# CNR-STIIMA-IRAS/rosdyn

Hardware: AMD Instinct MI355X
Metric: RNEA+regressor evals/s (6-DOF, batch 1e6) (higher is better)
Workload: dtype f64; 1 GPU; configs[1]: 6-DOF chain (ur10_like base_link->wrist_3_link, n=6, P=60), batch 1000000 samples per GPU, fp64 getJointTorque + dense getRegressor, inputs sample-major, Y layout stacked; samples_per_gpu=1000000, n_active=6, n_params=60, parallelism=sample-sharded x1

## Files before the change

### rosdyn_amd/csrc/rdyn_kernels.hip

```cpp
#include <hip/hip_runtime.h>
#include <type_traits>
#include "rdyn_device.h"
#include "rdyn_devmath.h"
#include "rdyn_kernels.h"
#include "rdyn_record_stage.h"

namespace
{

enum
{
  MODE_REGRESSOR = 0,
  MODE_TORQUE = 1,
  MODE_INERTIA = 2,
  MODE_REGRESSOR_GRAM = 3,
  MODE_REGRESSOR_EXPAND = 4,
  MODE_REGRESSOR_EXPAND_STAGED = 5
};
#define RDYN_IS_EXPAND(MODE) ((MODE) == MODE_REGRESSOR_EXPAND || (MODE) == MODE_REGRESSOR_EXPAND_STAGED)
#define RDYN_IS_REGRESSOR(MODE) ((MODE) == MODE_REGRESSOR || (MODE) == MODE_REGRESSOR_GRAM || RDYN_IS_EXPAND(MODE))
#define RDYN_BODY_EXIT return

#ifdef RDYN_LOCAL_WAVES
#define RDYN_LOCAL_ATTR __attribute__((amdgpu_waves_per_eu(RDYN_LOCAL_WAVES, RDYN_LOCAL_WAVES)))
#else
#define RDYN_LOCAL_ATTR
#endif
template <int NJ, int MODE>
__global__ __launch_bounds__(256) RDYN_LOCAL_ATTR void k_local_sweep(const RdynSweepArgs a)
{
  const unsigned blk = blockIdx.x;
  constexpr double* expand_tile = nullptr;
#include "rdyn_local_sweep_body.inc"
}
template <int NJ, int MODE>
__global__ __launch_bounds__(64) RDYN_LOCAL_ATTR void k_local_sweep_rec(const RdynSweepArgs a)
{
  const unsigned blk = blockIdx.x;
  constexpr double* expand_tile = nullptr;
#define RDYN_LOCAL_WGS 64
#include "rdyn_local_sweep_body.inc"
}
#ifndef RDYN_EXPAND_WAVES
#define RDYN_EXPAND_WAVES 2
#endif
template <int NJ>
__global__ __launch_bounds__(64) __attribute__((amdgpu_waves_per_eu(RDYN_EXPAND_WAVES, RDYN_EXPAND_WAVES))) void k_expand_staged(const RdynSweepArgs a)
{
  constexpr int MODE = MODE_REGRESSOR_EXPAND_STAGED;
  extern __shared__ __attribute__((aligned(16))) double expand_tile[];
  const unsigned blk = blockIdx.x;
#include "rdyn_local_sweep_body.inc"
}

template <int NJ, int MODE>
__global__ __launch_bounds__(256) void k_local_sweep_multi(const RdynSweepArgs* __restrict__ table)
{
#pragma clang diagnostic push
#pragma clang diagnostic ignored "-Wold-style-cast"
  const RDYN_CONST_AS RdynSweepArgs& a = *((const RDYN_CONST_AS RdynSweepArgs*)table + blockIdx.y);
#pragma clang diagnostic pop
  const unsigned blk = blockIdx.x;
  constexpr double* expand_tile = nullptr;
#include "rdyn_local_sweep_body.inc"
}

template <int NJ, int LEVEL, bool STAGED, class Args>
__device__ __forceinline__ void base_sweep_body(const Args& a, const int64_t s, char* lds = nullptr)
{
  ChainPtr c = as_const(a.chain);
  const int lane = threadIdx.x & 63;
  bool stg = false;
  RecordRing<96> ringT;
  RecordRing<48> ringV, ringA;
  char* small_area = nullptr;
  if constexpr (STAGED)
  {
    const int64_t s_wave = s - lane;
    stg = a.n_samples - s_wave >= 64;
    if (stg)
    {
      char* p = lds;
      if (a.T_links)
      {
        ringT.init(p, a.T_links + s_wave * a.tl_ss, 96u * (NJ + 1), lane);
        p += RecordRing<96>::BYTES;
      }
      if (LEVEL >= 2 && a.twists)
      {
        ringV.init(p, a.twists + s_wave * a.tw_ss, 48u * (NJ + 1), lane);
        p += RecordRing<48>::BYTES;
      }
      if (LEVEL >= 3 && a.dtwists)
      {
        ringA.init(p, a.dtwists + s_wave * a.tw_ss, 48u * (NJ + 1), lane);
        p += RecordRing<48>::BYTES;
      }
      small_area = p;
    }
  }
  if (s >= a.n_samples) return;
  const double* __restrict__ qp = a.q + s * a.in_ss;
  const double* __restrict__ dqp = (LEVEL >= 2 && a.dq) ? a.dq + s * a.in_ss : nullptr;
  const double* __restrict__ ddqp = (LEVEL >= 3 && a.ddq) ? a.ddq + s * a.in_ss : nullptr;
  const int64_t es = a.out_se;

  double R[9] = {1, 0, 0, 0, 1, 0, 0, 0, 1};
  V3 p = mk(0, 0, 0);
  V3 vlin = mk(0, 0, 0), vang = mk(0, 0, 0), alin = mk(0, 0, 0), aang = mk(0, 0, 0);

  auto put3x4 = [&](double* __restrict__ o) {
#pragma unroll
    for (int cc = 0; cc < 3; ++cc)
#pragma unroll
      for (int r = 0; r < 3; ++r) o[(int64_t)(cc * 3 + r) * es] = R[r * 3 + cc];
    o[9 * es] = p.x;
    o[10 * es] = p.y;
    o[11 * es] = p.z;
  };
  auto put6 = [&](double* __restrict__ o, V3 l, V3 g) {
    o[0] = l.x; o[es] = l.y; o[2 * es] = l.z; o[3 * es] = g.x; o[4 * es] = g.y; o[5 * es] = g.z;
  };

  auto frame_out = [&](const int link) {
    if (!a.T_links) return;
    if (STAGED && stg)
    {
#pragma unroll
      for (int cc = 0; cc < 3; ++cc)
#pragma unroll
        for (int r = 0; r < 3; ++r) ringT.put((uint32_t)(96 * link + 8 * (cc * 3 + r)), R[r * 3 + cc]);
      ringT.put((uint32_t)(96 * link + 72), p.x);
      ringT.put((uint32_t)(96 * link + 80), p.y);
      ringT.put((uint32_t)(96 * link + 88), p.z);
      ringT.flush(96 * link, 96 * (link + 1));
    }
    else
      put3x4(a.T_links + s * a.tl_ss + (int64_t)(12 * link) * es);
  };
  auto six_out = [&](const RecordRing<48>& ring, double* base, const int link, V3 l, V3 g) {
    if (STAGED && stg)
    {
      ring.put((uint32_t)(48 * link), l.x);
      ring.put((uint32_t)(48 * link + 8), l.y);
      ring.put((uint32_t)(48 * link + 16), l.z);
      ring.put((uint32_t)(48 * link + 24), g.x);
      ring.put((uint32_t)(48 * link + 32), g.y);
      ring.put((uint32_t)(48 * link + 40), g.z);
      ring.flush(48 * link, 48 * (link + 1));
    }
    else
      put6(base + s * a.tw_ss + (int64_t)(6 * link) * es, l, g);
  };
  V3 pref = mk(0, 0, 0);
  int j_up = 0;
  const bool jst = LEVEL == 1 && STAGED && stg && a.J;
  SmallRecords smJ;
  V3 zs[(LEVEL == 1 && STAGED) ? NJ : 1], pos[(LEVEL == 1 && STAGED) ? NJ : 1];
  if (LEVEL == 1 && !STAGED && a.J)
  {
    double R1[9] = {1, 0, 0, 0, 1, 0, 0, 0, 1};
    V3 p1 = mk(0, 0, 0);
#pragma unroll
    for (int l = 0; l < NJ; ++l)
    {
      JointRef J = c->j[l];
      if (l < a.j_link)
      {
        if (J.in_idx >= 0) ++j_up;
        const double ql = J.in_idx >= 0 ? qp[J.in_idx * a.in_sj] : 0.0;
        double Rpc[9];
        V3 t = ld3(J.t);
        if (J.type == RDYN_REVOLUTE)
        {
          double sn, cs;
          rdyn_sincos(ql, &sn, &cs);
          const double oc = 1.0 - cs;
#pragma unroll
          for (int i = 0; i < 9; ++i) Rpc[i] = fma(sn, J.B[i], fma(oc, J.C[i], J.A[i]));
        }
        else
        {
#pragma unroll
          for (int i = 0; i < 9; ++i) Rpc[i] = J.A[i];
          if (J.type == RDYN_PRISMATIC) t = axpy(t, ld3(J.up), ql);
        }
        p1 = p1 + rot(R1, t);
        double Rn[9];
#pragma unroll
        for (int r = 0; r < 3; ++r)
#pragma unroll
          for (int cc = 0; cc < 3; ++cc)
            Rn[r * 3 + cc] = fma(R1[r * 3 + 0], Rpc[cc], fma(R1[r * 3 + 1], Rpc[3 + cc], R1[r * 3 + 2] * Rpc[6 + cc]));
#pragma unroll
        for (int i = 0; i < 9; ++i) R1[i] = Rn[i];
      }
    }
    pref = p1;
  }
  frame_out(0);
  if (LEVEL >= 2 && a.twists) six_out(ringV, a.twists, 0, vlin, vang);
  if (LEVEL >= 3 && a.dtwists) six_out(ringA, a.dtwists, 0, alin, aang);

#pragma unroll
  for (int f = 0; f < NJ; ++f)
  {
    JointRef J = c->j[f];
    const int type = J.type;
    const int idx = J.in_idx;
    double qf = 0.0, dqf = 0.0, ddqf = 0.0;
    if (idx >= 0)
    {
      const int64_t o = idx * a.in_sj;
      qf = qp[o];
      if (LEVEL >= 2 && dqp) dqf = dqp[o];
      if (LEVEL >= 3 && ddqp) ddqf = ddqp[o];
    }
    double Rpc[9];
    V3 t = ld3(J.t);
    if (type == RDYN_REVOLUTE)
    {
      double sn, cs;
      rdyn_sincos(qf, &sn, &cs);
      const double oc = 1.0 - cs;
#pragma unroll
      for (int i = 0; i < 9; ++i) Rpc[i] = fma(sn, J.B[i], fma(oc, J.C[i], J.A[i]));
    }
    else
    {
#pragma unroll
      for (int i = 0; i < 9; ++i) Rpc[i] = J.A[i];
      if (type == RDYN_PRISMATIC) t = axpy(t, ld3(J.up), qf);
    }
    const V3 zl = LEVEL >= 1 ? rot(R, ld3(J.up)) : mk(0, 0, 0);
    const V3 d = rot(R, t);
    double Rn[9];
#pragma unroll
    for (int r = 0; r < 3; ++r)
#pragma unroll
      for (int cc = 0; cc < 3; ++cc)
        Rn[r * 3 + cc] = fma(R[r * 3 + 0], Rpc[cc], fma(R[r * 3 + 1], Rpc[3 + cc], R[r * 3 + 2] * Rpc[6 + cc]));
#pragma unroll
    for (int i = 0; i < 9; ++i) R[i] = Rn[i];
    p = p + d;
    if (LEVEL == 1 && STAGED)
    {
      zs[(LEVEL == 1 && STAGED) ? f : 0] = zl;
      pos[(LEVEL == 1 && STAGED) ? f : 0] = p;
    }
    if (LEVEL == 1 && !STAGED && a.J && idx >= 0)
    {
      V3 jlin = mk(0, 0, 0), jang = mk(0, 0, 0);
      if (idx < j_up)
      {
        if (type == RDYN_REVOLUTE)
        {
          jlin = cross(zl, pref - p);
          jang = zl;
        }
        else if (type == RDYN_PRISMATIC)
          jlin = zl;
      }
      put6(a.J + s * a.j_ss + (int64_t)(6 * idx) * es, jlin, jang);
    }
    if (LEVEL >= 2)
    {
      V3 Sl = mk(0, 0, 0), Sa = mk(0, 0, 0);
      if (type == RDYN_REVOLUTE) Sa = zl;
      else if (type == RDYN_PRISMATIC) Sl = zl;
      const V3 nvl = axpy(vlin + cross(vang, d), Sl, dqf);
      const V3 nva = axpy(vang, Sa, dqf);
      if (LEVEL >= 3)
      {
        const V3 cl = cross(nva, Sl) + cross(nvl, Sa);
        const V3 ca = cross(nva, Sa);
        alin = axpy(axpy(alin + cross(aang, d), cl, dqf), Sl, ddqf);
        aang = axpy(axpy(aang, ca, dqf), Sa, ddqf);
      }
      vlin = nvl;
      vang = nva;
    }
    frame_out(f + 1);
    if (LEVEL >= 2 && a.twists) six_out(ringV, a.twists, f + 1, vlin, vang);
    if (LEVEL >= 3 && a.dtwists) six_out(ringA, a.dtwists, f + 1, alin, aang);
  }
  if (STAGED && stg)
  {
    if (a.T_links) ringT.finish();
    if (LEVEL >= 2 && a.twists) ringV.finish();
    if (LEVEL >= 3 && a.dtwists) ringA.finish();
  }
  SmallRecords sm;
  if (a.T_bt)
  {
    if (STAGED && stg)
    {
      sm.init(small_area, 12, lane);
#pragma unroll
      for (int cc = 0; cc < 3; ++cc)
#pragma unroll
        for (int r = 0; r < 3; ++r) sm.put(cc * 3 + r, R[r * 3 + cc]);
      sm.put(9, p.x);
      sm.put(10, p.y);
      sm.put(11, p.z);
      sm.copy_out(a.T_bt + (s - lane) * a.tb_ss, lane);
    }
    else
      put3x4(a.T_bt + s * a.tb_ss);
  }
  if constexpr (LEVEL == 1 && STAGED)
  {
    if (a.J)
    {
      if (jst) smJ.init(small_area, 6 * c->n_active, lane);
      V3 pr = p;
      int up = 0;
#pragma unroll
      for (int l = 0; l < NJ; ++l)
      {
        if (a.j_link == l + 1) pr = pos[l];
        if (l < a.j_link && c->j[l].in_idx >= 0) ++up;
      }
      if (a.j_link == 0) pr = mk(0, 0, 0);
#pragma unroll
      for (int l = 0; l < NJ; ++l)
      {
        const int k = c->j[l].in_idx;
        if (k < 0) continue;
        const int ty = c->j[l].type;
        V3 jlin = mk(0, 0, 0), jang = mk(0, 0, 0);
        if (k < up)
        {
          if (ty == RDYN_REVOLUTE)
          {
            jlin = cross(zs[l], pr - pos[l]);
            jang = zs[l];
          }
          else if (ty == RDYN_PRISMATIC)
            jlin = zs[l];
        }
        if (jst)
        {
          smJ.put(6 * k, jlin.x); smJ.put(6 * k + 1, jlin.y); smJ.put(6 * k + 2, jlin.z);
          smJ.put(6 * k + 3, jang.x); smJ.put(6 * k + 4, jang.y); smJ.put(6 * k + 5, jang.z);
        }
        else
          put6(a.J + s * a.j_ss + (int64_t)(6 * k) * es, jlin, jang);
      }
      if (jst) smJ.copy_out(a.J + (s - lane) * a.j_ss, lane);
    }
  }
}

template <int NJ, int LEVEL>
__global__ __launch_bounds__(256) void k_base_sweep(const RdynKinArgs a)
{
  base_sweep_body<NJ, LEVEL, false>(a, (int64_t)blockIdx.x * 256 + threadIdx.x);
}
template <int NJ, int LEVEL>
__global__ __launch_bounds__(64) void k_base_sweep_staged(const RdynKinArgs a)
{
  extern __shared__ __attribute__((aligned(16))) char stage_lds[];
  base_sweep_body<NJ, LEVEL, true>(a, (int64_t)blockIdx.x * 64 + threadIdx.x, stage_lds);
}

template <int NJ>
__global__ __launch_bounds__(256) void k_sample_all(const RdynAllArgs all)
{
  const unsigned blk = blockIdx.x;
  constexpr double* expand_tile = nullptr;
  switch (blockIdx.y)
  {
  case 0:
    if (all.frames.T_bt || all.frames.T_links) base_sweep_body<NJ, 0, false>(all.frames, (int64_t)blk * 256 + threadIdx.x);
    return;
  case 1:
    if (all.jacobian.J) base_sweep_body<NJ, 1, false>(all.jacobian, (int64_t)blk * 256 + threadIdx.x);
    return;
  case 2:
    if (all.twists.dtwists) base_sweep_body<NJ, 3, false>(all.twists, (int64_t)blk * 256 + threadIdx.x);
    else if (all.twists.twists) base_sweep_body<NJ, 2, false>(all.twists, (int64_t)blk * 256 + threadIdx.x);
    return;
  case 3:
  {
    if (!all.torque.tau) return;
    constexpr int MODE = MODE_TORQUE;
    const RdynSweepArgs& a = all.torque;
#include "rdyn_local_sweep_body.inc"
    return;
  }
  case 4:
  {
    if (!all.torque_nl.tau) return;
    constexpr int MODE = MODE_TORQUE;
    const RdynSweepArgs& a = all.torque_nl;
#include "rdyn_local_sweep_body.inc"
    return;
  }
  case 5:
  {
    if (!all.inertia.M) return;
    constexpr int MODE = MODE_INERTIA;
    const RdynSweepArgs& a = all.inertia;
#include "rdyn_local_sweep_body.inc"
    return;
  }
  default:
  {
    if (!all.regressor.Y) return;
    constexpr int MODE = MODE_REGRESSOR;
    const RdynSweepArgs& a = all.regressor;
#include "rdyn_local_sweep_body.inc"
    return;
  }
  }
}

template <int NJ>
hipError_t launch_local_nj(int mode, const RdynSweepArgs& a, hipStream_t st)
{
  const unsigned grid = (unsigned)((a.n_samples + 255) / 256);
  switch (mode)
  {
  case MODE_REGRESSOR_EXPAND_STAGED:
    hipLaunchKernelGGL((k_expand_staged<NJ>), dim3((unsigned)((a.n_samples + 63) / 64)), dim3(64), (size_t)64 * (RDYN_EXPAND_TILE_COLS(NJ) * NJ + 2 + 3 * NJ + 1) * sizeof(double), st, a);
    break;
  case MODE_REGRESSOR: hipLaunchKernelGGL((k_local_sweep<NJ, MODE_REGRESSOR>), dim3(grid), dim3(256), 0, st, a); break;
  case MODE_REGRESSOR_GRAM: hipLaunchKernelGGL((k_local_sweep<NJ, MODE_REGRESSOR_GRAM>), dim3(grid), dim3(256), 0, st, a); break;
  case MODE_REGRESSOR_EXPAND: hipLaunchKernelGGL((k_local_sweep<NJ, MODE_REGRESSOR_EXPAND>), dim3(grid), dim3(256), 0, st, a); break;
  case MODE_TORQUE:
    if (a.staged) hipLaunchKernelGGL((k_local_sweep_rec<NJ, MODE_TORQUE>), dim3((unsigned)((a.n_samples + 63) / 64)), dim3(64), (size_t)64 * (a.staged | 1) * 8, st, a);
    else hipLaunchKernelGGL((k_local_sweep<NJ, MODE_TORQUE>), dim3(grid), dim3(256), 0, st, a);
    break;
  default:
    if (a.staged) hipLaunchKernelGGL((k_local_sweep_rec<NJ, MODE_INERTIA>), dim3((unsigned)((a.n_samples + 63) / 64)), dim3(64), (size_t)32 * (a.staged | 1) * 8, st, a);
    else hipLaunchKernelGGL((k_local_sweep<NJ, MODE_INERTIA>), dim3(grid), dim3(256), 0, st, a);
    break;
  }
  return hipGetLastError();
}
constexpr size_t kFramesStageLds = 33 * 1024;
template <int NJ>
hipError_t launch_base_nj(const RdynKinArgs& a, hipStream_t st)
{
  if (a.staged)
  {
    size_t lds = 0, small = 0;
    if (a.T_links) lds += RecordRing<96>::BYTES;
    if (a.twists) lds += RecordRing<48>::BYTES;
    if (a.dtwists) lds += RecordRing<48>::BYTES;
    if (a.T_bt) small = (size_t)64 * 13 * 8;
    if (a.J && (size_t)64 * (size_t)((6 * a.n_active) | 1) * 8 > small) small = (size_t)64 * (size_t)((6 * a.n_active) | 1) * 8;
    lds += small;
    if (a.T_links && lds < kFramesStageLds) lds = kFramesStageLds;
#ifdef RDYN_STAGE_LDS_PAD
    lds += RDYN_STAGE_LDS_PAD;
#endif
    const unsigned g64 = (unsigned)((a.n_samples + 63) / 64);
    if (a.dtwists) hipLaunchKernelGGL((k_base_sweep_staged<NJ, 3>), dim3(g64), dim3(64), lds, st, a);
    else if (a.twists) hipLaunchKernelGGL((k_base_sweep_staged<NJ, 2>), dim3(g64), dim3(64), lds, st, a);
    else if (a.J) hipLaunchKernelGGL((k_base_sweep_staged<NJ, 1>), dim3(g64), dim3(64), lds, st, a);
    else hipLaunchKernelGGL((k_base_sweep_staged<NJ, 0>), dim3(g64), dim3(64), lds, st, a);
    return hipGetLastError();
  }
  const unsigned grid = (unsigned)((a.n_samples + 255) / 256);
  if (a.dtwists) hipLaunchKernelGGL((k_base_sweep<NJ, 3>), dim3(grid), dim3(256), 0, st, a);
  else if (a.twists) hipLaunchKernelGGL((k_base_sweep<NJ, 2>), dim3(grid), dim3(256), 0, st, a);
  else if (a.J) hipLaunchKernelGGL((k_base_sweep<NJ, 1>), dim3(grid), dim3(256), 0, st, a);
#ifdef RDYN_BASE0_LDS_PAD
  else hipLaunchKernelGGL((k_base_sweep<NJ, 0>), dim3(grid), dim3(256), RDYN_BASE0_LDS_PAD, st, a);
#else
  else hipLaunchKernelGGL((k_base_sweep<NJ, 0>), dim3(grid), dim3(256), 0, st, a);
#endif
  return hipGetLastError();
}

}

#define RDYN_DISPATCH_NJ(nj, CALL)                 \
  switch (nj)                                      \
  {                                                \
  case 1: return CALL(1);                          \
  case 2: return CALL(2);                          \
  case 3: return CALL(3);                          \
  case 4: return CALL(4);                          \
  case 5: return CALL(5);                          \
  case 6: return CALL(6);                          \
  case 7: return CALL(7);                          \
  case 8: return CALL(8);                          \
  case 9: return CALL(9);                          \
  case 10: return CALL(10);                        \
  default: return hipErrorInvalidValue;            \
  }

#ifndef RDYN_KERNELS_PART
#error "compile with -DRDYN_KERNELS_PART=<0..3>"
#endif
#if RDYN_KERNELS_PART == 0
hipError_t rdyn_launch_local_sweep(int n_joints, int mode, const RdynSweepArgs& a, hipStream_t st)
{
  if (a.n_samples <= 0) return hipSuccess;
#define CALL(N) launch_local_nj<N>(mode, a, st)
  RDYN_DISPATCH_NJ(n_joints, CALL)
#undef CALL
}
#endif

#if RDYN_KERNELS_PART == 1
namespace
{
template <int NJ>
hipError_t launch_all_nj(const RdynAllArgs& a, hipStream_t st)
{
  hipLaunchKernelGGL((k_sample_all<NJ>), dim3((unsigned)((a.n_samples + 255) / 256), 7), dim3(256), 0, st, a);
  return hipGetLastError();
}
}
hipError_t rdyn_launch_sample_all(int n_joints, const RdynAllArgs& a, hipStream_t st)
{
  if (a.n_samples <= 0) return hipSuccess;
#define CALL(N) launch_all_nj<N>(a, st)
  RDYN_DISPATCH_NJ(n_joints, CALL)
#undef CALL
}
#endif

#if RDYN_KERNELS_PART == 2
static hipError_t launch_base_dispatch(int n_joints, const RdynKinArgs& a, hipStream_t st)
{
#define CALL(N) launch_base_nj<N>(a, st)
  RDYN_DISPATCH_NJ(n_joints, CALL)
#undef CALL
}
hipError_t rdyn_launch_base_sweep(int n_joints, const RdynKinArgs& a, hipStream_t st)
{
  if (a.n_samples <= 0) return hipSuccess;
  if (a.J && (a.twists || a.dtwists || a.T_bt || a.T_links))
  {
    RdynKinArgs j = a, rest = a;
    j.twists = j.dtwists = j.T_bt = j.T_links = nullptr;
    rest.J = nullptr;
    const hipError_t e = launch_base_dispatch(n_joints, j, st);
    if (e != hipSuccess) return e;
    return launch_base_dispatch(n_joints, rest, st);
  }
  return launch_base_dispatch(n_joints, a, st);
}
#endif

#if RDYN_KERNELS_PART == 3
namespace
{
template <int NJ>
hipError_t launch_local_multi_nj(int mode, const RdynSweepArgs* table, int n_items, int64_t max_samples, hipStream_t st)
{
  const dim3 grid((unsigned)((max_samples + 255) / 256), (unsigned)n_items);
  switch (mode)
  {
  case MODE_REGRESSOR: hipLaunchKernelGGL((k_local_sweep_multi<NJ, MODE_REGRESSOR>), grid, dim3(256), 0, st, table); break;
  case MODE_TORQUE: hipLaunchKernelGGL((k_local_sweep_multi<NJ, MODE_TORQUE>), grid, dim3(256), 0, st, table); break;
  default: hipLaunchKernelGGL((k_local_sweep_multi<NJ, MODE_INERTIA>), grid, dim3(256), 0, st, table); break;
  }
  return hipGetLastError();
}
}

hipError_t rdyn_launch_local_sweep_multi(int n_joints, int mode, const RdynSweepArgs* table, int n_items, int64_t max_samples, hipStream_t st)
{
  if (n_items <= 0 || max_samples <= 0) return hipSuccess;
#define CALL(N) launch_local_multi_nj<N>(mode, table, n_items, max_samples, st)
  RDYN_DISPATCH_NJ(n_joints, CALL)
#undef CALL
}
#endif
```

Before: 1.889 billion evals/s.

## Add specialized torque RNEA kernel with LDS-parked link wrenches and hoisted trig

Adds a dedicated torque-only RNEA kernel instead of reusing the generic local sweep body. It loads all joint inputs and computes sincos up front, keeps the per-link spatial quantities inline, and parks the forward-pass wrenches of the first few links in LDS to cut register pressure. The backward pass then reads them back. The cost is extra LDS traffic and a second code path to maintain. The benchmark metric is the regressor plus torque pair, so only the torque part is affected.

```diff
diff --git a/rosdyn_amd/csrc/rdyn_kernels.hip b/rosdyn_amd/csrc/rdyn_kernels.hip
--- a/rosdyn_amd/csrc/rdyn_kernels.hip
+++ b/rosdyn_amd/csrc/rdyn_kernels.hip
@@ -40,6 +40,29 @@
   constexpr double* expand_tile = nullptr;
 #define RDYN_LOCAL_WGS 64
 #include "rdyn_local_sweep_body.inc"
+}
+#ifdef RDYN_TORQUE_WAVES
+#define RDYN_TORQUE_ATTR __attribute__((amdgpu_waves_per_eu(RDYN_TORQUE_WAVES, RDYN_TORQUE_WAVES)))
+#else
+#define RDYN_TORQUE_ATTR
+#endif
+#ifndef RDYN_TORQUE_PARK_MAX
+#define RDYN_TORQUE_PARK_MAX 3
+#endif
+constexpr int torque_parked_links(int nj) { return nj - 1 < RDYN_TORQUE_PARK_MAX ? nj - 1 : RDYN_TORQUE_PARK_MAX; }
+template <int NJ>
+__global__ __launch_bounds__(256) RDYN_TORQUE_ATTR void k_torque_sweep(const RdynSweepArgs a)
+{
+  const unsigned blk = blockIdx.x;
+#define RDYN_TORQUE_WGS 256
+#include "rdyn_torque_sweep_body.inc"
+}
+template <int NJ>
+__global__ __launch_bounds__(64) RDYN_TORQUE_ATTR void k_torque_sweep_rec(const RdynSweepArgs a)
+{
+  const unsigned blk = blockIdx.x;
+#define RDYN_TORQUE_WGS 64
+#include "rdyn_torque_sweep_body.inc"
 }
 #ifndef RDYN_EXPAND_WAVES
 #define RDYN_EXPAND_WAVES 2
@@ -429,8 +452,12 @@
   case MODE_REGRESSOR_GRAM: hipLaunchKernelGGL((k_local_sweep<NJ, MODE_REGRESSOR_GRAM>), dim3(grid), dim3(256), 0, st, a); break;
   case MODE_REGRESSOR_EXPAND: hipLaunchKernelGGL((k_local_sweep<NJ, MODE_REGRESSOR_EXPAND>), dim3(grid), dim3(256), 0, st, a); break;
   case MODE_TORQUE:
-    if (a.staged) hipLaunchKernelGGL((k_local_sweep_rec<NJ, MODE_TORQUE>), dim3((unsigned)((a.n_samples + 63) / 64)), dim3(64), (size_t)64 * (a.staged | 1) * 8, st, a);
-    else hipLaunchKernelGGL((k_local_sweep<NJ, MODE_TORQUE>), dim3(grid), dim3(256), 0, st, a);
+    if (a.staged)
+    {
+      const size_t tile = (size_t)64 * (a.staged | 1) * 8, parked = (size_t)torque_parked_links(NJ) * 6 * 64 * 8;
+      hipLaunchKernelGGL((k_torque_sweep_rec<NJ>), dim3((unsigned)((a.n_samples + 63) / 64)), dim3(64), tile > parked ? tile : parked, st, a);
+    }
+    else hipLaunchKernelGGL((k_torque_sweep<NJ>), dim3(grid), dim3(256), 0, st, a);
     break;
   default:
     if (a.staged) hipLaunchKernelGGL((k_local_sweep_rec<NJ, MODE_INERTIA>), dim3((unsigned)((a.n_samples + 63) / 64)), dim3(64), (size_t)32 * (a.staged | 1) * 8, st, a);
diff --git a/rosdyn_amd/csrc/rdyn_torque_sweep_body.inc b/rosdyn_amd/csrc/rdyn_torque_sweep_body.inc
--- /dev/null
+++ b/rosdyn_amd/csrc/rdyn_torque_sweep_body.inc
@@ -0,0 +1,251 @@
+#ifndef RDYN_TORQUE_HOIST
+#define RDYN_TORQUE_HOIST 1
+#endif
+  ChainPtr c = as_const(a.chain);
+  constexpr int WGS = RDYN_TORQUE_WGS;
+  constexpr int PARK = torque_parked_links(NJ);
+  static_assert(PARK >= 0 && PARK * 6 * 64 * 8 <= 10240 && PARK < (NJ > 1 ? NJ : 2), "parked links");
+#if RDYN_TORQUE_WGS == 64
+  extern __shared__ __attribute__((aligned(16))) double tq_park[];
+#else
+  __shared__ double tq_park[(PARK ? PARK : 1) * 6 * WGS];
+#endif
+  double* const park = tq_park + threadIdx.x;
+
+  const int64_t s = (int64_t)blk * WGS + threadIdx.x;
+  if (s >= a.n_samples) return;
+  const double* __restrict__ qp = a.q + s * a.in_ss;
+  const double* __restrict__ dqp = a.dq ? a.dq + s * a.in_ss : nullptr;
+  const double* __restrict__ ddqp = a.ddq ? a.ddq + s * a.in_ss : nullptr;
+
+  double qin[NJ], dqin[NJ], ddqin[NJ];
+  double sv0[NJ], sv1[NJ];
+#if RDYN_TORQUE_HOIST
+#pragma unroll
+  for (int f = 0; f < NJ; ++f)
+  {
+    const int idx = c->j[f].in_idx;
+    const double v = qp[(idx >= 0 ? idx : 0) * a.in_sj];
+    qin[f] = idx >= 0 ? v : 0.0;
+  }
+#pragma unroll
+  for (int f = 0; f < NJ; ++f) dqin[f] = 0.0;
+  if (dqp)
+  {
+#pragma unroll
+    for (int f = 0; f < NJ; ++f)
+    {
+      const int idx = c->j[f].in_idx;
+      const double v = dqp[(idx >= 0 ? idx : 0) * a.in_sj];
+      dqin[f] = idx >= 0 ? v : 0.0;
+    }
+  }
+#pragma unroll
+  for (int f = 0; f < NJ; ++f) ddqin[f] = 0.0;
+  if (ddqp)
+  {
+#pragma unroll
+    for (int f = 0; f < NJ; ++f)
+    {
+      const int idx = c->j[f].in_idx;
+      const double v = ddqp[(idx >= 0 ? idx : 0) * a.in_sj];
+      ddqin[f] = idx >= 0 ? v : 0.0;
+    }
+  }
+  {
+    bool big = false;
+#pragma unroll
+    for (int f = 0; f < NJ; ++f)
+    {
+      double sn, cs;
+      rdyn_sincos_small(qin[f], &sn, &cs);
+      sv0[f] = sn;
+      sv1[f] = 1.0 - cs;
+      big = big || (c->j[f].type == RDYN_REVOLUTE && !(fabs(qin[f]) <= 1048576.0));
+    }
+    if (__builtin_expect(big, 0))
+    {
+#pragma unroll
+      for (int f = 0; f < NJ; ++f)
+      {
+        if (c->j[f].type == RDYN_REVOLUTE && !(fabs(qin[f]) <= 1048576.0))
+        {
+          double sn, cs;
+          sincos(qin[f], &sn, &cs);
+          sv0[f] = sn;
+          sv1[f] = 1.0 - cs;
+        }
+      }
+    }
+#pragma unroll
+    for (int f = 0; f < NJ; ++f)
+    {
+      if (c->j[f].type != RDYN_REVOLUTE)
+      {
+        sv0[f] = qin[f];
+        sv1[f] = 0.0;
+      }
+    }
+  }
+#endif
+
+  V3 w = mk(0, 0, 0), vl = mk(0, 0, 0), al = mk(0, 0, 0);
+  V3 acc = mk(-c->g[0], -c->g[1], -c->g[2]);
+  V3 pl = mk(0, 0, 0);
+  V3 Fo[NJ], No[NJ];
+  double tau[NJ];
+#pragma unroll
+  for (int l = 0; l < NJ; ++l) tau[l] = 0.0;
+
+#pragma unroll
+  for (int f = 0; f < NJ; ++f)
+  {
+    JointRef J = c->j[f];
+    const int type = J.type;
+#if !RDYN_TORQUE_HOIST
+    const int idx = J.in_idx;
+    qin[f] = dqin[f] = ddqin[f] = 0.0;
+    if (idx >= 0)
+    {
+      const int64_t o = idx * a.in_sj;
+      qin[f] = qp[o];
+      if (dqp) dqin[f] = dqp[o];
+      if (ddqp) ddqin[f] = ddqp[o];
+    }
+    if (type == RDYN_REVOLUTE)
+    {
+      double sn, cs;
+      rdyn_sincos(qin[f], &sn, &cs);
+      sv0[f] = sn;
+      sv1[f] = 1.0 - cs;
+    }
+    else
+    {
+      sv0[f] = qin[f];
+      sv1[f] = 0.0;
+    }
+#endif
+    const double dqf = dqin[f], ddqf = ddqin[f];
+    double R[9];
+    V3 t = ld3(J.t);
+    if (type == RDYN_REVOLUTE)
+    {
+#pragma unroll
+      for (int i = 0; i < 9; ++i) R[i] = fma(sv0[f], J.B[i], fma(sv1[f], J.C[i], J.A[i]));
+    }
+    else
+    {
+#pragma unroll
+      for (int i = 0; i < 9; ++i) R[i] = J.A[i];
+      if (type == RDYN_PRISMATIC) t = axpy(t, ld3(J.up), sv0[f]);
+    }
+    {
+      const V3 wn = rotT(R, w);
+      const V3 vn = rotT(R, vl + cross(w, t));
+      const V3 aln = rotT(R, al);
+      const V3 an = rotT(R, acc + cross(al, t));
+      w = wn; vl = vn; al = aln; acc = an;
+    }
+    const V3 u = ld3(J.u);
+    if (type == RDYN_REVOLUTE)
+    {
+      acc = axpy(acc, cross(vl, u), dqf);
+      al = axpy(axpy(al, cross(w, u), dqf), u, ddqf);
+      w = axpy(w, u, dqf);
+    }
+    else if (type == RDYN_PRISMATIC)
+    {
+      acc = axpy(axpy(acc, cross(w, u), dqf), u, ddqf);
+      vl = axpy(vl, u, dqf);
+    }
+    const RDYN_CONST_AS double* pi = J.pi;
+    const double m = pi[0];
+    const V3 h = ld3(pi + 1);
+    const V3 d = acc + cross(w, vl);
+    V3 fo = axpy(cross(al, h) + cross(w, cross(w, h)), d, m);
+    V3 no = symv(pi + 4, al) + cross(w, symv(pi + 4, w)) + cross(h, d);
+    if (a.ext)
+    {
+      pl = rotT(R, pl + t);
+      const double* __restrict__ ep = a.ext + s * a.ext_ss + (int64_t)(6 * (f + 1)) * a.ext_se;
+      const V3 el = mk(ep[0], ep[a.ext_se], ep[2 * a.ext_se]);
+      const V3 ea = mk(ep[3 * a.ext_se], ep[4 * a.ext_se], ep[5 * a.ext_se]);
+      fo = fo - (el + cross(ea, pl));
+      no = no - ea;
+    }
+    if (f < PARK)
+    {
+      park[(6 * f + 0) * WGS] = fo.x; park[(6 * f + 1) * WGS] = fo.y; park[(6 * f + 2) * WGS] = fo.z;
+      park[(6 * f + 3) * WGS] = no.x; park[(6 * f + 4) * WGS] = no.y; park[(6 * f + 5) * WGS] = no.z;
+    }
+    else
+    {
+      Fo[f] = fo;
+      No[f] = no;
+    }
+  }
+
+  {
+    V3 F = mk(0, 0, 0), N = mk(0, 0, 0);
+#pragma unroll
+    for (int f = NJ - 1; f >= 0; --f)
+    {
+      JointRef J = c->j[f];
+      const int type = J.type;
+      if (f < PARK)
+      {
+        F = F + mk(park[(6 * f + 0) * WGS], park[(6 * f + 1) * WGS], park[(6 * f + 2) * WGS]);
+        N = N + mk(park[(6 * f + 3) * WGS], park[(6 * f + 4) * WGS], park[(6 * f + 5) * WGS]);
+      }
+      else
+      {
+        F = F + Fo[f];
+        N = N + No[f];
+      }
+      const V3 u = ld3(J.u);
+      if (type == RDYN_REVOLUTE) tau[f] = dot(u, N);
+      else if (type == RDYN_PRISMATIC) tau[f] = dot(u, F);
+      if (f == 0) break;
+      double R[9];
+      V3 t = ld3(J.t);
+      if (type == RDYN_REVOLUTE)
+      {
+#pragma unroll
+        for (int i = 0; i < 9; ++i) R[i] = fma(sv0[f], J.B[i], fma(sv1[f], J.C[i], J.A[i]));
+      }
+      else
+      {
+#pragma unroll
+        for (int i = 0; i < 9; ++i) R[i] = J.A[i];
+        if (type == RDYN_PRISMATIC) t = axpy(t, ld3(J.up), sv0[f]);
+      }
+      const V3 Fp = rot(R, F);
+      N = rot(R, N) + cross(t, Fp);
+      F = Fp;
+    }
+  }
+
+  bool stg_rec = false;
+  SmallRecords sm;
+#if RDYN_TORQUE_WGS == 64
+  if (a.staged && a.n_samples - (s - threadIdx.x) >= 64)
+  {
+    rs_wave_fence();
+    sm.init((char*)tq_park, c->n_active, threadIdx.x);
+    stg_rec = true;
+  }
+#endif
+  if (a.tau)
+  {
+    double* __restrict__ tp = a.tau + s * a.tau_ss;
+#pragma unroll
+    for (int l = 0; l < NJ; ++l)
+    {
+      const int r = c->j[l].in_idx;
+      if (r < 0) continue;
+      if (stg_rec) sm.put(r, tau[l]);
+      else tp[r * a.tau_sj] = tau[l];
+    }
+    if (stg_rec) sm.copy_out(a.tau + (s - threadIdx.x) * a.tau_ss, threadIdx.x);
+  }
+#undef RDYN_TORQUE_WGS
```

New measurement: 1.892 billion evals/s, median of 4. No clear change (+0.2%).
